# MiloszKrajewski/K4os.Compression.LZ4

Measured on AMD Instinct MI355X. Metric: GiB/s encode+decode on batched 64 KiB blocks; bit-exact vs C# ref, higher is better.
Workload: dtype u8

## Files before the change

k4os/compression/lz4_amd/csrc/k4lz4_capi.hip:

```cpp
#include <hip/hip_runtime.h>
#include <stdint.h>
#include <stdio.h>
#include <stdlib.h>
#include <string.h>
#include <algorithm>
#include <atomic>
#include <memory>
#include <new>
#include <condition_variable>
#include <functional>
#include <map>
#include <mutex>
#include <string>
#include <thread>
#include <chrono>
#include <vector>

#include "../../../../include/k4lz4.h"
#include "k4lz4_decode.hpp"
#include "k4lz4_encode_fast.hpp"
#include "k4lz4_parse.hpp"
#include "k4lz4_pickle.hpp"
#include "k4lz4_segments.hpp"
#include "k4lz4_encode_hc.hpp"
// ... 62 lines not shown
    hipEvent_t ev_up[MAX_PARTS] = {}, ev_len[MAX_PARTS] = {};
    uint8_t *h_len = nullptr; size_t h_len_cap = 0;
    struct Pool *pool = nullptr, *pool_dl = nullptr;
    bool pool_failed = false, pool_dl_failed = false;
    int stage_threads = 7;
    uint32_t *d_pace = nullptr;
    uint32_t *d_status = nullptr;
    int split_pct = -1;
    bool no_pair = false;
    int direct_span_pct = 200;
    bool no_direct = false;
    int lds_floor_per_cu = 8;
    int cost_pct = 48;
    int dec_parts = 4, dec_parts_direct = 8;
    int last_decode_kernel = 0;
    int hop2_max_per_cu = 12;
    bool hc_cand_lds = true;
    int hc_cand_dynlds = 0;
    int hc_segs = 0;
    bool hc_chain_parts = true;
    int hc_mem_pct = 33;
    int pace_min_per_cu = 6;
    bool use_pace = true;
    bool prof_gtab = false;
    uint8_t *d_parse = nullptr; size_t d_parse_cap = 0;
    bool use_parse = true;
    bool parse_queue = false;
    bool hc_records = true;
    bool parse_seg = true;
    bool parse_big = true;
    bool parse_persist = true;
    bool parse_inline_emit = true;
    bool parse_migrate = true;
    bool parse_pcost = false;
    int parse_waves = 16;
    bool trace = false;
    std::vector<uint8_t> h_chain;
    uint8_t *d_chain = nullptr; size_t d_chain_cap = 0;
    hipEvent_t ev_chain = nullptr;
    uint8_t *d_fr = nullptr; size_t d_fr_cap = 0;
    uint8_t *d_fb = nullptr; size_t d_fb_cap = 0;
    uint8_t *d_lg = nullptr; size_t d_lg_cap = 0;
    uint8_t *d_frd = nullptr; size_t d_frd_cap = 0;
    uint8_t *d_lgr = nullptr; size_t d_lgr_cap = 0;
    uint8_t *d_lga = nullptr; size_t d_lga_cap = 0;
    std::vector<uint8_t> h_fw;
    uint8_t *d_fw = nullptr; size_t d_fw_cap = 0;
    hipEvent_t ev_fw = nullptr;
    struct DictScratch {
        std::vector<uint8_t> host;
        uint8_t *dev = nullptr; size_t cap = 0;
        hipEvent_t ev = nullptr;
        std::vector<uint32_t> table, kept;
    } dict_fast, dict_hc;
    uint8_t *d_dpick = nullptr; size_t d_dpick_cap = 0;
};

struct k4lz4_dict_set {
    struct Family {
        bool on = false;
        uint64_t *toff = nullptr, *eoff = nullptr;
        uint32_t *tlen = nullptr, *elen = nullptr, *etab = nullptr;
        uint8_t *tables = nullptr;
        std::vector<uint32_t> table, kept;
        int64_t ntables = 0, loads = 0;
    };
    int device = -1;
// ... 413 lines not shown
                K4_HIP(ctx, hipStreamSynchronize(stream));
                K4_HIP(ctx, hipStreamSynchronize(ctx->aux2));
            }
            int rc = grow(ctx, &ctx->d_seg, &ctx->d_seg_cap, total, false);
            if (rc == K4LZ4_OK) rc = grow(ctx, &ctx->d_seg_first, &ctx->d_seg_first_cap, (size_t)cnt * 4, false);
            if (rc != K4LZ4_OK) return rc;
            sg.hdr = (k4::SegHdr *)ctx->d_seg; sg.items = (k4::SegItem *)(ctx->d_seg + o_items); sg.work = (uint32_t *)(ctx->d_seg + o_work);
            sg.blocks = (uint32_t *)(ctx->d_seg + o_blocks); sg.snaps = (uint32_t *)(ctx->d_seg + o_snaps); sg.tables = (uint32_t *)(ctx->d_seg + o_tables);
            sg.first = (int32_t *)ctx->d_seg_first;
            sg.seg_min = ctx->seg_min; sg.seg_target = ctx->seg_target; sg.seg_warm = ctx->seg_warm; sg.seg_div = ctx->seg_div; sg.seg_target_max = ctx->seg_target_max; sg.spin_max = ctx->seg_spin_max; sg.max_items = (uint32_t)max_items;
            hipLaunchKernelGGL(k4::k4_seg_plan_kernel, dim3(1), dim3(256), 0, stream, a, sg);
            a.seg_first = sg.first; a.seg_items = sg.items; a.seg_snaps = sg.snaps;
            seg = true;
        }
        auto segments_start = [&]() -> int {
            if (!seg) return K4LZ4_OK;
            K4_HIP(ctx, hipEventRecord(ctx->ev_fork, stream));
            K4_HIP(ctx, hipStreamWaitEvent(ctx->aux2, ctx->ev_fork, 0));
            hipLaunchKernelGGL(k4::k4_encode_seg_kernel, dim3((unsigned)((sg.max_items + k4::ENCODE_WAVES_PER_WG - 1) / k4::ENCODE_WAVES_PER_WG)), dim3(64 * k4::ENCODE_WAVES_PER_WG), 0, ctx->aux2, a, sg);
            K4_HIP(ctx, hipEventRecord(ctx->ev_join2, ctx->aux2));
            return K4LZ4_OK;
        };
        auto segments_join = [&]() -> int {
            if (!seg) return K4LZ4_OK;
            K4_HIP(ctx, hipStreamWaitEvent(stream, ctx->ev_join2, 0));
            hipLaunchKernelGGL(k4::k4_seg_join_kernel, dim3((unsigned)std::min<int64_t>(k4::SEG_MAX_BLOCKS, cnt)), dim3(64), 0, stream, a, sg);
            return K4LZ4_OK;
        };
        if (dd && dd->dict) {
            a.dict = dd->dict; a.dictOff = dd->off + first; a.dictLen = dd->len + first;
            a.dictMode = dd->mode ? dd->mode + first : nullptr;
        }
        if (reorder && parse_path && kind == KIND_ENCODE && ctx->parse_pcost) {
            a.cost = d_cost; a.hist = d_hist; a.order_out = d_order;
            K4_HIP(ctx, hipMemsetAsync(d_hist, 0, 2 * k4::PCOST_BUCKETS * 4, stream));
            hipLaunchKernelGGL(k4::k4_pcost_kernel, dim3((unsigned)((cnt + k4::PCOST_WAVES_PER_WG - 1) / k4::PCOST_WAVES_PER_WG)), dim3(64 * k4::PCOST_WAVES_PER_WG), 0, stream, a);
            hipLaunchKernelGGL(k4::k4_porder_kernel, dim3((unsigned)((cnt + 255) / 256)), dim3(256), 0, stream, a);
            a.order = d_order;
        }
        else if (reorder) {
            a.cost = d_cost; a.hist = d_hist; a.order_out = d_order;
            K4_HIP(ctx, hipMemsetAsync(d_hist, 0, (2 * k4::COST_BUCKETS + 16) * 4, stream));
            hipLaunchKernelGGL(k4::k4_cost_kernel, dim3((unsigned)cnt), dim3(64), 0, stream, a, encode_like ? 0 : 1,
                               kind == KIND_ENCODE && parse_path ? k4::COST_SAMPLE_PARSE : k4::COST_SAMPLE);
            const bool two_kernels = kind == KIND_ENCODE && !a.prof && cnt > 512 && !(flags & K4LZ4_FLAG_NO_SPLIT) &&
                                     cnt > 8 * (int64_t)ctx->cu_count && ctx->split_pct <= 0;
            k4::BatchArgs ao = a;
            ao.first = two_kernels ? (uint32_t)ctx->cost_pct : 0u;
            ao.total = (uint32_t)((int64_t)ctx->lds_floor_per_cu * (int64_t)ctx->cu_count);
            hipLaunchKernelGGL(k4::k4_order_kernel, dim3((unsigned)((cnt + 255) / 256)), dim3(256), 0, stream, ao, (uint32_t)lds_share(ctx, cnt));
            a.order = d_order;
            if (two_kernels) a.split = d_hist + 2 * k4::COST_BUCKETS;
        }
        const unsigned wg4 = (unsigned)((cnt + k4::DECODE_WAVES_PER_WG - 1) / k4::DECODE_WAVES_PER_WG);
        bool parse_here = kind == KIND_ENCODE && (parse_path || (parse_seg_path && (a.order || cnt == 1)));
        const bool big_ok = ctx->parse_big && ctx->parse_inline_emit;
        bool any_small = true, any_big = big_ok;
        if (parse_here && hostLen) {
            any_small = false; any_big = false;
            for (int64_t i = 0; i < cnt && !(any_small && (any_big || !big_ok)); i++) {
                const int32_t len = hostLen[first + i];
                if (len >= (int32_t)k4::PARSE_MIN_LEN && len < k4::LIMIT_64K) any_small = true;
                else if (len >= k4::LIMIT_64K && big_ok) any_big = true;
            }
            parse_here = any_small || any_big;
        }
        int64_t waves = 0, nwg = 0, nwg_seg = 0;
        const bool seg_two_step = seg && parse_here && parse_seg_path;
        bool queue = false, slot_recs = false;
        size_t o_meta = 0, o_gtab = 0;
// ... 1761 lines not shown
    if (e == hipSuccess) e = hipStreamCreateWithFlags(&ctx->dlq, hipStreamNonBlocking);
    if (const char *pct = getenv("K4LZ4_SPLIT_PCT")) { const int v = atoi(pct); ctx->split_pct = v < 1 ? 1 : (v > 100 ? 100 : v); }
    ctx->no_pair = getenv("K4LZ4_NO_PAIR") != nullptr;
    ctx->prof_gtab = getenv("K4LZ4_PROF_GTAB") != nullptr;
    ctx->use_pace = getenv("K4LZ4_NO_PACE") == nullptr;
    if (const char *e = getenv("K4LZ4_PACE_MIN")) ctx->pace_min_per_cu = std::max(0, atoi(e));
    if (const char *e = getenv("K4LZ4_DIRECT_SPAN_PCT")) ctx->direct_span_pct = std::max(100, atoi(e));
    if (const char *e = getenv("K4LZ4_NO_DIRECT")) ctx->no_direct = atoi(e) != 0;
    if (const char *e = getenv("K4LZ4_LDS_FLOOR")) ctx->lds_floor_per_cu = std::max(0, std::min(8, atoi(e)));
    if (const char *e = getenv("K4LZ4_COST_PCT")) ctx->cost_pct = std::max(1, std::min(99, atoi(e)));
    if (const char *e = getenv("K4LZ4_DEC_PARTS")) ctx->dec_parts = std::max(2, std::min(MAX_PARTS, atoi(e)));
    if (const char *e = getenv("K4LZ4_DEC_PARTS_DIRECT")) ctx->dec_parts_direct = std::max(2, std::min(MAX_PARTS, atoi(e)));
    if (const char *e = getenv("K4LZ4_HOP2_MAX")) ctx->hop2_max_per_cu = std::max(0, atoi(e));
    ctx->hc_chain_parts = getenv("K4LZ4_HC_CHAIN_OLD") == nullptr;
    ctx->hc_cand_lds = getenv("K4LZ4_HC_CAND_MEM") == nullptr;
    if (const char *e = getenv("K4LZ4_HC_CAND_DYNLDS")) ctx->hc_cand_dynlds = std::max(0, std::min(65536, atoi(e)));
    if (const char *e = getenv("K4LZ4_HC_SEGS")) { const int v = atoi(e); ctx->hc_segs = v >= 4 ? 4 : (v >= 2 ? 2 : (v == 1 ? 1 : 0)); }
    if (const char *e = getenv("K4LZ4_HC_MEM_PCT")) ctx->hc_mem_pct = std::max(0, std::min(100, atoi(e)));
    ctx->use_segments = getenv("K4LZ4_NO_SEGMENTS") == nullptr;
    if (const char *e = getenv("K4LZ4_SEG_MIN")) ctx->seg_min = (uint32_t)std::max(65536 + 4096, atoi(e));
    if (const char *e = getenv("K4LZ4_SEG_TARGET")) ctx->seg_target = ctx->seg_target_max = (uint32_t)std::max(8192, atoi(e));
    if (const char *e = getenv("K4LZ4_SEG_TARGET_MAX")) ctx->seg_target_max = (uint32_t)std::max(8192, atoi(e));
    if (const char *e = getenv("K4LZ4_SEG_WARM")) ctx->seg_warm = (uint32_t)std::max(0, atoi(e));
    if (const char *e = getenv("K4LZ4_SEG_SPIN_MAX")) ctx->seg_spin_max = (uint32_t)std::max(0, atoi(e));
    if (const char *e = getenv("K4LZ4_SEG_DIV")) ctx->seg_div = (uint32_t)std::max(0, atoi(e));
    if (const char *e = getenv("K4LZ4_PICKLE_SPLIT_MIN")) ctx->pickle_split_min = std::max(0, atoi(e));
    if (const char *e = getenv("K4LZ4_STAGE_THREADS")) ctx->stage_threads = std::max(0, std::min(63, atoi(e) - 1));
    ctx->use_parse = getenv("K4LZ4_NO_PARSE") == nullptr;
    ctx->parse_queue = getenv("K4LZ4_PARSE_QUEUE") != nullptr;
    ctx->parse_persist = getenv("K4LZ4_NO_PERSIST") == nullptr;
    ctx->parse_big = getenv("K4LZ4_NO_PARSE_BIG") == nullptr;
    ctx->parse_seg = getenv("K4LZ4_NO_PARSE_SEG") == nullptr;
    ctx->hc_records = getenv("K4LZ4_NO_HC_RECORDS") == nullptr;
    ctx->parse_pcost = getenv("K4LZ4_PCOST") != nullptr;
    ctx->parse_migrate = getenv("K4LZ4_NO_MIGRATE") == nullptr;
    ctx->parse_inline_emit = getenv("K4LZ4_NO_INLINE_EMIT") == nullptr;
    if (const char *e = getenv("K4LZ4_PARSE_WAVES")) ctx->parse_waves = std::max(1, std::min(k4::PARSE_MAX_WAVES, atoi(e)));
    ctx->trace = getenv("K4LZ4_TRACE") != nullptr;
    if (e != hipSuccess) { delete ctx; return hip_fail(nullptr, e, "hipStreamCreate"); }
    *out = ctx;
    return K4LZ4_OK;
}

void k4lz4_ctx_destroy(k4lz4_ctx *ctx)
{
    if (!ctx) return;
    (void)hipSetDevice(ctx->device);
    if (ctx->stream) { (void)hipStreamSynchronize(ctx->stream); (void)hipStreamDestroy(ctx->stream); }
    if (ctx->aux) { (void)hipStreamSynchronize(ctx->aux); (void)hipStreamDestroy(ctx->aux); }
    if (ctx->aux2) { (void)hipStreamSynchronize(ctx->aux2); (void)hipStreamDestroy(ctx->aux2); }
    if (ctx->ev_join2) (void)hipEventDestroy(ctx->ev_join2);
    if (ctx->d_seg) (void)hipFree(ctx->d_seg);
    if (ctx->d_seg_first) (void)hipFree(ctx->d_seg_first);
    if (ctx->ev_fork) (void)hipEventDestroy(ctx->ev_fork);
    if (ctx->ev_join) (void)hipEventDestroy(ctx->ev_join);
    if (ctx->ev_busy) (void)hipEventDestroy(ctx->ev_busy);
    for (int b = 0; b < 2; b++) {
        if (ctx->ev_in[b]) (void)hipEventDestroy(ctx->ev_in[b]);
        if (ctx->ev_out[b]) (void)hipEventDestroy(ctx->ev_out[b]);
        if (ctx->h_in[b]) (void)hipHostFree(ctx->h_in[b]);
        if (ctx->h_out[b]) (void)hipHostFree(ctx->h_out[b]);
    }
    if (ctx->d_pack) (void)hipFree(ctx->d_pack);
    if (ctx->h_len) (void)hipHostFree(ctx->h_len);
    for (int b = 0; b < MAX_PARTS; b++) {
        if (ctx->ev_up[b]) (void)hipEventDestroy(ctx->ev_up[b]);
        if (ctx->ev_len[b]) (void)hipEventDestroy(ctx->ev_len[b]);
// ... 2436 lines not shown
```

k4os/compression/lz4_amd/csrc/k4lz4_encode_fast.hpp:

```cpp
#pragma once
#include "k4lz4_common.hpp"

namespace k4 {

#ifndef K4_SEG_WAVES_MIN
#define K4_SEG_WAVES_MIN 5
#endif
#ifndef K4_GTAB_DUTY
#define K4_GTAB_DUTY 3
#endif
#ifndef K4_PACE
#define K4_PACE 1
#endif

template <int TYPE> struct FastTable;

template <> struct FastTable<1> {
    uint16_t *t;
    __device__ __forceinline__ static uint32_t hash(const uint8_t *p) { return (ld32u(p) * 2654435761u) >> (32 - 13); }
    __device__ __forceinline__ static uint32_t hash_of(uint32_t seq, uint32_t) { return (seq * 2654435761u) >> (32 - 13); }
    __device__ __forceinline__ uint32_t get(uint32_t h) const { return t[h]; }
    __device__ __forceinline__ void put(uint32_t h, uint32_t pos) const { t[h] = (uint16_t)pos; }
    __device__ __forceinline__ uint32_t get_nt(uint32_t h) const
    {
// ... 750 lines not shown
        op += last_run;
    }
    if (seq_count) *seq_count = sequences;
    if (sr) { sr->stop = U; sr->state = 2u; }
    if (PROF && pc && lane == 0) {
        pc[0] = prof_now<PROF>() - t_begin; pc[1] = c_probe; pc[2] = c_ext; pc[3] = c_emit;
        pc[4] = n_seq; pc[5] = n_round; pc[6] = n_dup; pc[7] = n_rt3;
        pc[11] = c_s1; pc[12] = c_s2; pc[13] = c_s3; pc[14] = c_s4; pc[15] = n_cont;
    }
    prof_place<PROF>(pc, 9, lane);
    return (int)op;
}

template <bool PAIRS = true, bool MORE = false, bool N2 = true, bool GTAB = false>
__device__ __forceinline__ int compress_fast_block(const uint8_t *src, int src_len, uint8_t *dst, int dst_cap,
                                                   int accel, uint32_t *ldsw, int lane, uint32_t *gtab = nullptr, bool x32 = false,
                                                   uint32_t *pace = nullptr, SegRun *sr = nullptr)
{
    const uint32_t a = accel < 1 ? 1u : (accel > 65536 ? 65536u : (uint32_t)accel);
    if (src_len < LIMIT_64K) return encode_fast_block<true, false, false, PAIRS, MORE, N2, GTAB>(src, src_len, dst, dst_cap, a, ldsw, lane, nullptr, false, nullptr, gtab, pace);
    if (x32) return encode_fast_block<false, false, true, PAIRS, MORE, N2, GTAB>(src, src_len, dst, dst_cap, a, ldsw, lane, nullptr, false, nullptr, gtab, pace, sr);
    return encode_fast_block<false, false, false, PAIRS, MORE, N2, GTAB>(src, src_len, dst, dst_cap, a, ldsw, lane, nullptr, false, nullptr, gtab, pace, sr);
}

__device__ __forceinline__ int codec_encode_result(int src_len, int ret, int flags)
{
    if (flags & FLAG_RAW_RETURN) return ret;
    if (src_len <= 0) return 0;
    return ret <= 0 ? -1 : ret;
}

constexpr int COST_SAMPLE = 512, COST_SAMPLE_PARSE = 256;
constexpr int COST_BUCKETS = 64;

__device__ __forceinline__ uint32_t cost_bucket(unsigned long long cost)
{
    if (cost < 4ull) return (uint32_t)cost;
    const uint32_t l = 63u - (uint32_t)__clzll(cost);
    const uint32_t bkt = 2u * l + (uint32_t)((cost >> (l - 1u)) & 1ull);
    return bkt < (uint32_t)COST_BUCKETS ? bkt : (uint32_t)COST_BUCKETS - 1u;
}

__global__ __launch_bounds__(64) void k4_cost_kernel(BatchArgs a, int by_length, int sample_bytes = COST_SAMPLE)
{
    __shared__ __attribute__((aligned(16))) uint32_t tab[ENCODE_LDS_DWORDS];
    const int lane = lane_id();
    const long long b = (long long)blockIdx.x;
    const int src_len = a.srcLen[b];
    unsigned long long cost = 0;
    if (src_len > 0) {
        if (by_length || src_len <= 64) {
            cost = (unsigned long long)src_len;
        } else {
            const int sample = src_len < sample_bytes ? src_len : sample_bytes;
            uint32_t nseq = 0;
            (void)encode_fast_block<true>(a.src + a.srcOff[b], sample, nullptr, 0x7fffffff, 1u, tab, lane, nullptr, true, &nseq);
            cost = ((unsigned long long)(nseq * 8u + (uint32_t)sample / 16u) * (unsigned long long)src_len) / (unsigned long long)sample;
        }
    }
    if (lane == 0) {
        const uint32_t bkt = cost_bucket(cost);
        a.cost[b] = bkt;
        atomicAdd(&a.hist[bkt], 1u);
    }
}

__device__ __forceinline__ unsigned long long bucket_cost(uint32_t bkt)
{
    if (bkt < 4u) return bkt ? (unsigned long long)bkt * 4ull : 1ull;
    const uint32_t l = bkt >> 1;
    return ((bkt & 1u) ? 7ull : 5ull) << (l - 1u);
}

__global__ __launch_bounds__(256) void k4_order_kernel(BatchArgs a, uint32_t lds_max = 0xffffffffu)
{
    if (blockIdx.x == 0 && threadIdx.x == 0 && a.first != 0u) {
        unsigned long long all = 0;
        for (uint32_t k = 0; k < (uint32_t)COST_BUCKETS; k++) all += (unsigned long long)a.hist[k] * bucket_cost(k);
        const unsigned long long want = all / 100ull * (unsigned long long)a.first;
        unsigned long long have = 0, cnt = 0;
        for (int k = COST_BUCKETS - 1; k >= 0 && have < want; k--) {
            const unsigned long long c = a.hist[k], w = bucket_cost((uint32_t)k);
            if (have + c * w <= want) { have += c * w; cnt += c; }
            else { const unsigned long long part = (want - have + w - 1ull) / w; cnt += part; have = want; }
        }
        const unsigned long long floor_n = (unsigned long long)a.total < (unsigned long long)a.n ? (unsigned long long)a.total : (unsigned long long)a.n;
        if (cnt < floor_n) cnt = floor_n;
        if (cnt > (unsigned long long)a.n) cnt = (unsigned long long)a.n;
        if (cnt > (unsigned long long)lds_max) cnt = (unsigned long long)lds_max;
        a.hist[2 * COST_BUCKETS] = (uint32_t)cnt;
    }
    const long long b = (long long)blockIdx.x * 256 + threadIdx.x;
    if (b >= a.n) return;
    const uint32_t bkt = a.cost[b];
    uint32_t before = 0;
    for (uint32_t k = bkt + 1u; k < (uint32_t)COST_BUCKETS; k++) before += a.hist[k];
    const uint32_t pos = before + atomicAdd(&a.hist[COST_BUCKETS + bkt], 1u);
    a.order_out[pos] = (uint32_t)b;
}

constexpr int ENCODE_WAVES_PER_WG = 2;
struct SegFirst { SegRun run; uint32_t cap; bool cut; };
__device__ __forceinline__ SegFirst seg_first_of(const BatchArgs &a, long long b)
{
    SegFirst f;
    f.cut = false; f.cap = 0u;
    f.run.begin = 0u; f.run.emit_from = 0u; f.run.stop_at = SEG_NONE; f.run.snap_pub = nullptr; f.run.snap_chk = nullptr; f.run.resume = nullptr;
    f.run.cut = 0u; f.run.stop = 0u; f.run.state = 3u; f.run.spin_max = 0u; f.run.fix = nullptr;
    if (!a.seg_first) return f;
    const int32_t it = (int32_t)uni((uint32_t)a.seg_first[b]);
    if (it < 0) return f;
    const uint32_t *w = (const uint32_t *)a.seg_items + SEG_ITEM_WORDS * (uint32_t)it;
    f.cut = true;
    f.run.spin_max = uni(((const uint32_t *)a.seg_items)[-(int)SEG_HDR_DWORDS + 3]);
    f.run.stop_at = uni(w[4]);
    f.cap = f.run.stop_at;
    f.run.snap_chk = a.seg_snaps + (size_t)(it + 1) * SEG_SNAP_DWORDS;
    f.run.fix = a.seg_snaps + (size_t)uni(((const uint32_t *)a.seg_items)[-(int)SEG_HDR_DWORDS + 7]) * SEG_SNAP_DWORDS + 4096ull * (unsigned long long)it;
    return f;
}
__device__ __forceinline__ void seg_first_done(const BatchArgs &a, long long b, const SegFirst &f, int ret, int lane)
{
    if (!f.cut || lane != 0) return;
    uint32_t *w = (uint32_t *)a.seg_items + SEG_ITEM_WORDS * (uint32_t)a.seg_first[b];
    w[6] = f.run.cut; w[7] = f.run.stop; w[8] = ret > 0 ? f.run.state : 3u; w[9] = (uint32_t)ret;
}

template <bool MORE, bool SEG = false>
__device__ __forceinline__ void encode_fast_kernel_body(const BatchArgs &a, uint32_t (*tabs)[ENCODE_LDS_DWORDS])
{
    const int lane = lane_id();
// ... 101 lines not shown
```

k4os/compression/lz4_amd/csrc/k4lz4_parse.hpp:

```cpp
#pragma once
#include "k4lz4_encode_fast.hpp"
#include <type_traits>
#ifdef K4_PARSE_DEBUG
#include <stdio.h>
#include <stdlib.h>
#endif

namespace k4 {

#ifndef K4_PARSE_K
#define K4_PARSE_K 1
#endif

constexpr uint32_t PARSE_REC_STRIDE = 16448u;
static_assert(PARSE_REC_STRIDE >= ((uint32_t)LIMIT_64K - 1u - 6u) / 4u + 1u + 62u, "a block below LIMIT_64K has at most (LIMIT_64K - 1 - 6) / 4 sequences; a round adds at most 64 / 4 + 1");
constexpr uint32_t PARSE_MIN_LEN = 128u;
constexpr uint32_t PARSE_REST = 0xffffffffu;
constexpr uint32_t PARSE_BIG = 0xfffffffeu;
constexpr int PARSE_MAX_WAVES = 16;
constexpr int PARSE_LDS_TABLES = 9;
constexpr int PARSE_SEEN_DWORDS = 128;

constexpr int PARSE_LDS_DWORDS = 4096 * PARSE_LDS_TABLES + PARSE_SEEN_DWORDS * PARSE_MAX_WAVES + 4;

// ... 34 lines not shown
}

__device__ __forceinline__ uint32_t ext28(const uint32_t *x)
{
    uint32_t acc = min((uint32_t)(__ffs((int)x[6]) - 1), 32u);
#pragma unroll
    for (int i = 5; i >= 0; i--) {
        const uint32_t t = min((uint32_t)(__ffs((int)x[i]) - 1), 32u);
        acc = t + (t == 32u ? acc : 0u);
    }
    return acc >> 3;
}

__device__ __forceinline__ void rec_store(uint2 *r, uint32_t x, uint32_t y)
{
#if defined(K4_NT_RECS) && !defined(K4_HOST_EMU)
    __builtin_nontemporal_store((((unsigned long long)y) << 32) | x, (unsigned long long *)r);
#else
    *r = make_uint2(x, y);
#endif
}
__device__ __forceinline__ uint2 rec_load(const uint2 *r)
{
#if defined(K4_NT_RECS) && !defined(K4_HOST_EMU)
    const unsigned long long v = __builtin_nontemporal_load((const unsigned long long *)r);
    return make_uint2((uint32_t)v, (uint32_t)(v >> 32));
#else
    return *r;
#endif
}

constexpr uint32_t HOP_LONG = 0x100u, HOP_LAZY = 0x200u, HOP_END = 0x400u, HOP_INVALID = 0x800u, HOP_TABMISS = 0x1000u;

struct ParseStats { uint32_t rounds, slow, groups, lazies, longs; };
constexpr int PARSE_FLUSH = -2;

struct ParseCtl {
    uint32_t *free_slots;
    uint32_t rec_cap;
    int claimed;
    bool resume;
    uint32_t c, sbase, sj, nrec, long_seen, long_rounds;
    bool test, more;
    uint32_t cut_pos;
    bool dry, stopped;
};

template <int K, bool GT, bool DRY = false, int TT = 1, bool SEG = false>
__device__ __forceinline__ uint32_t parse_block(const uint8_t *src, const uint32_t U, uint2 *recs, void *tabv, uint32_t *seen, const int lane, unsigned long long *pc = nullptr,
                                                ParseStats *stats = nullptr, ParseCtl *ctl = nullptr, SegRun *sr = nullptr)
{
    static_assert(!SEG || (TT != 1 && K == 1 && !DRY), "segments: byU32 blocks, one sub-window per round");
    typedef FastTable<TT> Table;
    static_assert(TT == 1 || K == 1, "byU32 tables: one sub-window per round");
    constexpr bool U32 = TT != 1;
    Table tab;
    tab.t = (decltype(tab.t))tabv;
    constexpr uint32_t SEEN_SHIFT = TT == 1 ? 1u : 0u;
    ParseStats st = {0u, 0u, 0u, 0u, 0u};
#define K4_ST(field, v) do { if (DRY) st.field += (v); } while (0)
#ifdef K4_PARSE_PROF
    unsigned long long pt[8] = {0, 0, 0, 0, 0, 0, 0, 0}, pn[8] = {0, 0, 0, 0, 0, 0, 0, 0}, plast = 0;
    const unsigned long long pbegin = prof_now<true>();
#define K4_PT(i) do { const unsigned long long t_ = prof_now<true>(); pt[i] += t_ - plast; plast = t_; } while (0)
#define K4_PN(i, v) (pn[i] += (v))
#define K4_TIC() const unsigned long long tic_ = (unsigned long long)__builtin_readcyclecounter()
#define K4_TOC(i) (pt[i] += (unsigned long long)__builtin_readcyclecounter() - tic_)
#else
#define K4_TIC() ((void)0)
#define K4_TOC(i) ((void)0)
#define K4_PT(i) ((void)0)
#define K4_PN(i, v) ((void)0)
#endif
#if defined(K4_PARSE_PROF) && !defined(K4_PARSE_PROF_SPLIT)
#define K4_TICA() K4_TIC()
#define K4_TOCA(i) K4_TOC(i)
#else
#define K4_TICA() ((void)0)
#define K4_TOCA(i) ((void)0)
#endif
#if defined(K4_PARSE_PROF) && defined(K4_PARSE_PROF_SPLIT)
#define K4_TICB() const unsigned long long ticb_ = (unsigned long long)__builtin_readcyclecounter()
#define K4_TOCB(i) (pt[i] += (unsigned long long)__builtin_readcyclecounter() - ticb_)
#define K4_TICC() const unsigned long long ticc_ = (unsigned long long)__builtin_readcyclecounter()
#define K4_TOCC(i) (pt[i] += (unsigned long long)__builtin_readcyclecounter() - ticc_)
#else
#define K4_TICB() ((void)0)
#define K4_TOCB(i) ((void)0)
#define K4_TICC() ((void)0)
#define K4_TOCC(i) ((void)0)
#endif
    const uint32_t mfl1 = U - (uint32_t)MFLIMIT + 1u;
// ... 671 lines not shown
    for (;;) {
        if (SEG) {
            cut_hit = uni(cut_hit ? 1u : 0u) != 0u;
            if (cut_hit) {
                cut_hit = false;
                if (handle_cut()) { ctl->stopped = true; return nrec; }
            }
            cut_pos = uni(cut_pos); nrec = uni(nrec); dry = uni(dry ? 1u : 0u) != 0u;
            c = uni(c); sbase = uni(sbase);
        }
        if (U32 && rec_cap && nrec + 64u * (uint32_t)K + 2u > rec_cap) {
            ctl->c = c; ctl->sbase = sbase; ctl->sj = sj; ctl->nrec = nrec; ctl->test = test; ctl->more = more;
            ctl->long_seen = long_seen; ctl->long_rounds = long_rounds;
            if (SEG) { ctl->cut_pos = cut_pos; ctl->dry = dry; }
            ctl->claimed = PARSE_FLUSH;
            return nrec;
        }
        if (GT && ctl && ctl->free_slots && (++mig_tick & 15u) == 0u) {
            const uint32_t fs = uni(lds_peek(ctl->free_slots));
            if (fs) {
                const uint32_t sl = (uint32_t)__ffs((int)fs) - 1u;
                uint32_t old = 0u;
                if (lane == 0) old = atomicAnd(ctl->free_slots, ~(1u << sl));
                if (uni(old) & (1u << sl)) {
                    ctl->c = c; ctl->sbase = sbase; ctl->sj = sj; ctl->nrec = nrec; ctl->test = test; ctl->more = more;
                    ctl->long_seen = long_seen; ctl->long_rounds = long_rounds;
                    if (SEG) { ctl->cut_pos = cut_pos; ctl->dry = dry; }
                    ctl->claimed = (int)sl;
                    wave_sync();
                    return nrec;
                }
            }
        }
        const bool plain = sj == 0u && c + 64u * (uint32_t)K + 28u <= U;
        if (K == 1 && plain && c + 63u <= sbase + 65u) {
            if (more && c + 108u <= U) { if (!fast_round(std::true_type{})) break; }
            else if (!fast_round(std::false_type{})) break;
        }
        else if (plain) { if (!round(std::true_type{})) break; }
        else if (!round(std::false_type{})) break;
    }
#ifdef K4_PARSE_PROF
    if (pc && lane == 0) {
        pc[0] = prof_now<true>() - pbegin;
        for (int i = 0; i < 6; i++) pc[1 + i] = pt[i];
        pc[7] = (unsigned long long)nrec | (pn[4] << 32);
        pc[11] = pn[0] | (pn[6] << 32);
        pc[12] = pn[1] | (pn[2] << 32);
        pc[13] = (pt[6] & 0xffffffffull) | (pt[7] << 32);
        pc[10] = pn[7];
        pc[14] = pn[3] | (pn[5] << 32);
    }
#endif
    if (DRY && stats) *stats = st;
#undef K4_ST
    if (SEG) {
        if (uni(dry ? 1u : 0u) != 0u) {
            agent_publish(sr->snap_pub, SEG_NONE);
            sr->state = 3u;
            ctl->stopped = true;
            nrec = 0u;
        } else {
            sr->stop = U; sr->state = 2u;
        }
    }
    return nrec;
// ... 128 lines not shown
        const bool mine = a.accel == 1 && (U32 ? big : (src_len >= (int)PARSE_MIN_LEN && src_len < LIMIT_64K));
        if (!mine) {
            if (!U32 && lane == 0) {
                meta[0] = (big && p.big) ? PARSE_BIG : PARSE_REST; meta[1] = 0u;
                if (big && p.big && p.nbig) atomicAdd(p.nbig, 1u);
            }
        } else {
            uint32_t n = 0u;
            const int ret = parse_one<K, TT, false>(a, p, lds, seen, in_lds, wave, waves, lane, b, a.src + a.srcOff[b], src_len, a.dst + a.dstOff[b], a.dstCap[b], nullptr, &n);
            if (lane == 0) {
                meta[0] = n; meta[1] = 0u;
                if (p.inline_emit) a.outLen[b] = codec_encode_result(src_len, ret, a.flags);
            }
        }
        if (!p.queue) return;
    }
}


__global__ __launch_bounds__(64 * PARSE_MAX_WAVES) void k4_parse_kernel(BatchArgs a, ParseArgs p)
{
    __shared__ __attribute__((aligned(16))) uint32_t lds[PARSE_LDS_DWORDS];
    parse_kernel_body<K4_PARSE_K>(a, p, lds);
}

__global__ __launch_bounds__(64 * PARSE_MAX_WAVES) void k4_parse_big_kernel(BatchArgs a, ParseArgs p)
{
    __shared__ __attribute__((aligned(16))) uint32_t lds[PARSE_LDS_DWORDS];
    if (a.flags & FLAG_X32) parse_kernel_body<1, 2>(a, p, lds);
    else parse_kernel_body<1, 0>(a, p, lds);
}


constexpr uint32_t PCOST_SAMPLE = 3072u;
constexpr int PCOST_BUCKETS = 512;
constexpr int PCOST_WAVES_PER_WG = 8;

__device__ __forceinline__ uint32_t pcost_bucket(unsigned long long cost)
{
    if (cost < 256ull) return 0u;
    const uint32_t l = 63u - (uint32_t)__clzll((long long)cost);
    const uint32_t b = 16u * (l - 8u) + (uint32_t)((cost >> (l - 4u)) & 15ull) + 1u;
    return b < (uint32_t)PCOST_BUCKETS ? b : (uint32_t)PCOST_BUCKETS - 1u;
}

__global__ __launch_bounds__(64 * PCOST_WAVES_PER_WG) void k4_pcost_kernel(BatchArgs a)
{
    __shared__ __attribute__((aligned(16))) uint32_t lds[PCOST_WAVES_PER_WG][4096 + PARSE_SEEN_DWORDS];
    const int lane = lane_id();
    const uint32_t wave = uni(threadIdx.x >> 6);
    const long long b = (long long)blockIdx.x * PCOST_WAVES_PER_WG + (long long)wave;
    if (b >= a.n) return;
    const int src_len = a.srcLen[b];
    unsigned long long cost = 0ull;
    if (src_len >= (int)PARSE_MIN_LEN && src_len < LIMIT_64K) {
        const uint32_t sample = (uint32_t)src_len < PCOST_SAMPLE ? (uint32_t)src_len : PCOST_SAMPLE;
        ParseStats st;
        const uint32_t nseq = parse_block<1, false, true>(a.src + a.srcOff[b], sample, nullptr, (uint16_t *)lds[wave], lds[wave] + 4096, lane, nullptr, &st);
        const unsigned long long cyc = 6500ull * st.rounds + 3000ull * st.slow + 120ull * nseq + 150ull * st.groups + 480ull * st.lazies + 1500ull * st.longs;
        cost = cyc * (unsigned long long)(uint32_t)src_len / sample;
    } else if (src_len > 0) {
        cost = 120ull * (unsigned long long)(uint32_t)src_len;
    }
    if (lane == 0) {
        const uint32_t bkt = pcost_bucket(cost);
        a.cost[b] = bkt;
        atomicAdd(&a.hist[bkt], 1u);
    }
}

__global__ __launch_bounds__(256) void k4_porder_kernel(BatchArgs a)
{
    __shared__ uint32_t before[PCOST_BUCKETS];
    for (int k = (int)threadIdx.x; k < PCOST_BUCKETS; k += 256) before[k] = a.hist[k];
    __syncthreads();
    if (threadIdx.x == 0) {
        uint32_t acc = 0u;
        for (int k = PCOST_BUCKETS - 1; k >= 0; k--) { const uint32_t c = before[k]; before[k] = acc; acc += c; }
    }
    __syncthreads();
    const long long b = (long long)blockIdx.x * 256 + threadIdx.x;
    if (b >= a.n) return;
    const uint32_t bkt = a.cost[b];
    a.order_out[before[bkt] + atomicAdd(&a.hist[PCOST_BUCKETS + bkt], 1u)] = (uint32_t)b;
}


constexpr int EMIT_WAVES_PER_WG = 4;

template <bool HC, bool BIG>
__device__ __forceinline__ bool emit_records(const uint8_t *src, const uint32_t U, uint8_t *dst, const int dst_cap, const uint2 *recs, const uint32_t nseq, const int lane, EmitState &st)
{
    const bool limited = dst_cap < compress_bound((int)U);
    const uint64_t olimit = (uint64_t)(dst_cap < 0 ? 0 : dst_cap);
    uint32_t op = st.op, emitted_to = st.emitted_to;
    uint2 rn = make_uint2(0u, 0u);
    if ((uint32_t)lane < nseq) rn = rec_load(recs + lane);
    for (uint32_t base = 0u; base < nseq; base += 64u) {
        const uint32_t n = nseq - base < 64u ? nseq - base : 64u;
        const bool mine = (uint32_t)lane < n;
        const uint2 r = rn;
        if (base + 64u + (uint32_t)lane < nseq) rn = rec_load(recs + base + 64u + (uint32_t)lane);
        const uint32_t pos = r.x, cpos = r.x - (r.y & 0xffffu);
        uint32_t code = r.y >> 16;
        if (BIG) {
            unsigned long long lng = ballot(mine && code == 0xffffu);
            while (lng) {
                const int g = ctz64(lng);
                lng &= lng - 1ull;
                const uint32_t gp = readlane_u32(pos, g), gc = readlane_u32(cpos, g);
                const uint32_t full = wave_count(src + gp + (uint32_t)MINMATCH, src + gc + (uint32_t)MINMATCH, (U - (uint32_t)LASTLITERALS) - (gp + (uint32_t)MINMATCH), lane);
                if (lane == g) code = full;
            }
        }
        const uint32_t end = mine ? pos + (uint32_t)MINMATCH + code : 0u;
        const uint32_t prev = (uint32_t)__shfl_up((int)end, 1);
        const uint32_t ls = lane == 0 ? emitted_to : prev;
        const uint32_t lit0 = mine ? pos - ls : 0u;
// ... 140 lines not shown
```

Measured before the change: 61.55.

## Enable fitted parse-cost ordering by default with persistent cost kernel

Turns on the parse-based cost estimate for ordering encode work by default. It replaces the old pcost kernel with a persistent grid-stride kernel that uses LDS plus global-memory hash tables and a round cap. It also takes cost weights fitted offline from measured per-block timings and switches the order kernel to a wave-scan suffix count over fine buckets. The aim is to schedule expensive blocks first and reduce tail imbalance. The cost is an extra sampling pass before every encode, and the fitted weights may not carry over to other data.

```diff
diff --git a/experiments/parse_cost_order/fit.py b/experiments/parse_cost_order/fit.py
--- /dev/null
+++ b/experiments/parse_cost_order/fit.py
@@ -0,0 +1,68 @@
+import ctypes as C, os, sys, subprocess, numpy as np
+ROOT = os.path.dirname(os.path.dirname(os.path.dirname(os.path.abspath(__file__))))
+sys.path.insert(0, ROOT)
+WORK = sys.argv[1]
+from k4os.compression.lz4_amd import corpus
+so = os.path.join(WORK, "libstudy.so")
+lib = C.CDLL(so)
+n, bs = 4096, 65536
+cache = os.path.join(WORK, "blocks.npy")
+if os.path.exists(cache): blocks = np.load(cache)
+else:
+    blocks = corpus.silesia_like_blocks(n, bs, seed=2); np.save(cache, blocks)
+uidx = np.array([ci + 12 * t for ci in range(12) for t in range(32)])
+ub = np.ascontiguousarray(blocks[uidx])
+off = (np.arange(384, dtype=np.uint64) * bs); lens = np.full(384, bs, np.int32)
+def stats(o, l):
+    out = np.zeros((384, 8), np.uint32)
+    lib.study_stats(ub.ctypes.data_as(C.POINTER(C.c_uint8)), C.c_void_p(off.ctypes.data), C.c_void_p(lens.ctypes.data), C.c_longlong(384), C.c_uint32(o), C.c_uint32(l), C.c_void_p(out.ctypes.data), C.c_int(8), C.c_uint32(0))
+    return out[:, :6].astype(np.float64), out[:, 6].astype(np.float64)
+b = np.arange(n); u = (b % 12) * 32 + (b // 12) % 32
+ls = np.zeros(384); ln = np.zeros(384); ms = np.zeros(384); mn = np.zeros(384)
+for f in ("parent_blocks", "oracleP_blocks", "oracleQ_blocks"):
+    res = np.load(os.path.join(WORK, "%s.npy" % f))
+    for r in res:
+        d = (r[:, 1] - r[:, 0]) / 1e5; k = r[:, 2].astype(int)
+        np.add.at(ls, u[k == 4], d[k == 4]); np.add.at(ln, u[k == 4], 1)
+        np.add.at(ms, u[k != 4], d[k != 4]); np.add.at(mn, u[k != 4], 1)
+lds = np.where(ln > 0, ls / np.maximum(ln, 1), np.nan); mem = np.where(mn > 0, ms / np.maximum(mn, 1), np.nan)
+both = (ln >= 2) & (mn >= 2)
+ratio = np.median(mem[both] / lds[both]); print("ratio", ratio, "both", both.sum(), "lds known", (ln > 0).sum())
+truth = np.where(np.isnan(lds), mem / ratio, lds)
+np.save(os.path.join(WORK, "truth.npy"), truth)
+names = corpus.SILESIA_NAMES
+def evaluate(tag, est):
+    e = est[u] + 1e-9 * np.random.default_rng(0).random(n)
+    t = truth[u]
+    cut = np.sort(e)[::-1][2303]
+    inl = e >= cut
+    tail_mem = (t[~inl] * ratio).max(); tail_lds = t[inl].max()
+    tcut = np.sort(t)[::-1][2303]
+    mis = ((t >= tcut) & ~inl).sum()
+    from scipy.stats import spearmanr
+    rho = spearmanr(est, truth).correlation
+    print("%-28s rho %.3f misplaced %4d  tail mem %.3f lds %.3f  mem>2.7: %4d  mem>2.85: %4d" % (tag, rho, mis, tail_mem, tail_lds, (t[~inl] * ratio > 2.7).sum(), (t[~inl] * ratio > 2.85).sum()))
+evaluate("truth", truth)
+full, _ = stats(0, 65536)
+np.save(os.path.join(WORK, "full.npy"), full)
+for ci, nm in enumerate(names):
+    s = full[ci * 32:(ci + 1) * 32]
+    print("%-8s truth %.3f | rounds %6.0f slow %6.0f nseq %6.0f groups %6.0f lazies %6.0f longs %6.0f" % ((nm, truth[ci * 32:(ci + 1) * 32].mean()) + tuple(s.mean(0))))
+A = np.c_[full, np.ones(384)]
+w, *_ = np.linalg.lstsq(A, truth, rcond=None)
+print("fit full (ms per unit):", w, "resid rms", np.sqrt(((A @ w - truth) ** 2).mean()))
+from scipy.optimize import nnls
+w2, _ = nnls(A, truth); print("nnls:", w2, "rms", np.sqrt(((A @ w2 - truth) ** 2).mean()))
+evaluate("full stats, lstsq", A @ w)
+evaluate("full stats, nnls", A @ w2)
+evaluate("full stats, old pcost w", full @ np.array([6500, 3000, 120, 150, 480, 1500.]))
+evaluate("full rounds only", full[:, 0])
+for (o, l) in ((0, 256), (0, 512), (0, 1024), (0, 2048), (0, 3072), (32768, 512), (32768, 1024), (16384, 1024), (4096, 1024), (1024, 1024)):
+    s, sl = stats(o, l)
+    sc = s * (bs / sl)[:, None]
+    evaluate("sample %d+%d nnls-w" % (o, l), np.c_[sc, np.ones(384)] @ w2)
+    evaluate("sample %d+%d lstsq-w" % (o, l), np.c_[sc, np.ones(384)] @ w)
+    evaluate("sample %d+%d oldw" % (o, l), sc @ np.array([6500, 3000, 120, 150, 480, 1500.]))
+    As = np.c_[sc, np.ones(384)]; ws, _ = nnls(As, truth)
+    evaluate("sample %d+%d refit" % (o, l), As @ ws); print("    refit w", np.round(ws, 6))
+    np.save(os.path.join(WORK, "s_%d_%d.npy" % (o, l)), sc)
diff --git a/experiments/parse_cost_order/fit_stats.cpp b/experiments/parse_cost_order/fit_stats.cpp
--- /dev/null
+++ b/experiments/parse_cost_order/fit_stats.cpp
@@ -0,0 +1,30 @@
+#include "hip/hip_runtime.h"
+#include "k4lz4_decode.hpp"
+#include "k4lz4_encode_fast.hpp"
+#include "k4lz4_parse.hpp"
+#include <vector>
+
+namespace k4 {
+__global__ void stats_kernel(BatchArgs a, uint32_t off, uint32_t len, uint32_t *out, uint32_t cap = 0)
+{
+    __shared__ __attribute__((aligned(16))) uint32_t lds[PCOST_WAVES_PER_WG][4096 + PARSE_SEEN_DWORDS];
+    const int lane = lane_id();
+    const uint32_t wave = uni(threadIdx.x >> 6);
+    const long long b = (long long)blockIdx.x * PCOST_WAVES_PER_WG + (long long)wave;
+    if (b >= a.n) return;
+    const uint32_t src_len = (uint32_t)a.srcLen[b];
+    uint32_t o = off, s = len;
+    if (o + s > src_len) { o = 0; s = s < src_len ? s : src_len; }
+    ParseStats st; st.max_rounds = cap;
+    const uint32_t nseq = parse_block<1, false, true>(a.src + a.srcOff[b] + o, s, nullptr, (uint16_t *)lds[wave], lds[wave] + 4096, lane, nullptr, &st);
+    if (lane == 0) { uint32_t *w = out + 8 * b; w[0] = st.rounds; w[1] = st.slow; w[2] = nseq; w[3] = st.groups; w[4] = st.lazies; w[5] = st.longs; w[6] = st.covered; }
+}
+}
+
+extern "C" int study_stats(const uint8_t *src, const uint64_t *srcOff, const int32_t *srcLen, long long n, uint32_t off, uint32_t len, uint32_t *out, int threads, uint32_t cap)
+{
+    k4::BatchArgs a{};
+    a.src = src; a.srcOff = srcOff; a.srcLen = srcLen; a.n = n; a.accel = 1;
+    k4emu::launch_fn(dim3((unsigned)((n + k4::PCOST_WAVES_PER_WG - 1) / k4::PCOST_WAVES_PER_WG)), dim3(64 * k4::PCOST_WAVES_PER_WG), [=] { k4::stats_kernel(a, off, len, out, cap); }, threads);
+    return 0;
+}
diff --git a/experiments/parse_cost_order/rank_blocks.py b/experiments/parse_cost_order/rank_blocks.py
--- /dev/null
+++ b/experiments/parse_cost_order/rank_blocks.py
@@ -0,0 +1,26 @@
+#!/usr/bin/env python
+import sys
+import numpy as np
+res = np.load(sys.argv[1])
+reps, n, _ = res.shape
+b = np.arange(n)
+u = (b % 12) * 32 + (b // 12) % 32
+dur = (res[:, :, 1] - res[:, :, 0]) / 1e5
+k = res[:, :, 2].astype(int)
+lds_s = np.zeros(384); lds_n = np.zeros(384); mem_s = np.zeros(384); mem_n = np.zeros(384)
+for r in range(reps):
+    np.add.at(lds_s, u[k[r] == 4], dur[r][k[r] == 4]); np.add.at(lds_n, u[k[r] == 4], 1)
+    np.add.at(mem_s, u[k[r] != 4], dur[r][k[r] != 4]); np.add.at(mem_n, u[k[r] != 4], 1)
+lds = np.where(lds_n > 0, lds_s / np.maximum(lds_n, 1), np.nan)
+mem = np.where(mem_n > 0, mem_s / np.maximum(mem_n, 1), np.nan)
+both = (lds_n >= 2) & (mem_n >= 2)
+ratio = float(np.median(mem[both] / lds[both])) if both.any() else 1.17
+P = np.where(np.isnan(lds), mem / ratio, lds)
+Q = np.where(np.isnan(mem), lds * ratio, mem)
+print("unique blocks with LDS stamps %d, with others %d, with both %d; ratio other / LDS %.3f" % ((lds_n > 0).sum(), (mem_n > 0).sum(), both.sum(), ratio))
+for tag, est, path in (("P", P, sys.argv[2]), ("Q", Q, sys.argv[3])):
+    bkt = np.clip(np.round(est / (est.max() * 1.0001) * 63.0), 0, 63).astype(np.uint8)
+    bkt[u].tofile(path)
+    cut = np.sort(est[u])[::-1][2304 - 1]
+    print("%s: estimate ms min %.3f max %.3f; the 2304th most expensive block has %.3f; LDS share per class:" % (tag, est.min(), est.max(), cut),
+          " ".join("%d:%.2f" % (c, float((est[u][c::12] >= cut).mean())) for c in range(12)))
diff --git a/experiments/parse_cost_order/rank_from_stamp.py b/experiments/parse_cost_order/rank_from_stamp.py
--- /dev/null
+++ b/experiments/parse_cost_order/rank_from_stamp.py
@@ -0,0 +1,29 @@
+#!/usr/bin/env python
+import re, sys
+NAMES = ("dickens", "mozilla", "mr", "nci", "ooffice", "osdb", "reymont", "samba", "sao", "webster", "xml", "x-ray")
+lds, mem = {}, {}
+kern, on = None, False
+for line in open(sys.argv[1]):
+    if line.startswith("ENCODE"): on = True; continue
+    if line.startswith("DECODE"): on = False
+    if not on: continue
+    m = re.match(r"\s*kernel (\d+) blocks", line)
+    if m: kern = int(m.group(1)); continue
+    m = re.match(r"\s*(\S+)\s+n\s+(\d+)\s+start.*duration mean ([\d.]+)", line)
+    if m and kern is not None:
+        name, cnt, d = m.group(1), int(m.group(2)), float(m.group(3))
+        if kern == 4: lds[name] = (cnt, d)
+        elif kern in (5, 6):
+            c0, d0 = mem.get(name, (0, 0.0))
+            mem[name] = (c0 + cnt, (c0 * d0 + cnt * d) / (c0 + cnt))
+both = sorted(mem[k][1] - lds[k][1] for k in NAMES if k in lds and k in mem and lds[k][0] >= 8 and mem[k][0] >= 8)
+pen = both[len(both) // 2] if both else 0.4
+estA, estB = {}, {}
+for k in NAMES:
+    estA[k] = lds[k][1] if k in lds and lds[k][0] >= 8 else max(0.0, mem[k][1] - pen)
+    estB[k] = mem[k][1] if k in mem and mem[k][0] >= 8 else lds[k][1] + pen
+for tag, est in (("A", estA), ("B", estB)):
+    ranked = sorted(NAMES, key=lambda k: est[k])
+    rank = {k: i for i, k in enumerate(ranked)}
+    print("%s=%s" % (tag, ",".join(str(rank[k]) for k in NAMES)))
+    print("# %s penalty %.3f most expensive first: %s" % (tag, pen, "  ".join("%s %.3f" % (k, est[k]) for k in reversed(ranked))), file=sys.stderr)
diff --git a/experiments/parse_cost_order/stamp_dump.py b/experiments/parse_cost_order/stamp_dump.py
--- /dev/null
+++ b/experiments/parse_cost_order/stamp_dump.py
@@ -0,0 +1,43 @@
+#!/usr/bin/env python
+import os, sys
+import numpy as np
+import torch
+sys.path.insert(0, os.getcwd())
+from k4os.compression.lz4_amd import LZ4Codec, corpus
+from k4os.compression.lz4_amd.device import DeviceBatch, DeviceCodec
+
+out, reps = sys.argv[1], int(sys.argv[2]) if len(sys.argv) > 2 else 4
+n, bs = 4096, 65536
+blocks = corpus.silesia_like_blocks(n, bs, seed=2)
+dc = DeviceCodec(0)
+lens = np.full(n, bs, np.int32)
+off = np.arange(n, dtype=np.uint64) * bs
+src = DeviceBatch.from_host(blocks.reshape(-1), off, lens, dc.device)
+comp = DeviceBatch.empty_slots(np.full(n, LZ4Codec.MaximumOutputSize(bs)), dc.device)
+dc.encode(src, comp)
+torch.cuda.synchronize()
+res = []
+for rep in range(reps + 1):
+    _, c = dc.profile(4, src, comp)
+    torch.cuda.synchronize()
+    c = c.cpu().numpy().astype(np.float64)
+    if rep: res.append(np.stack([c[:, 8], c[:, 9], c[:, 11], c[:, 12]], axis=1))
+res = np.stack(res)
+np.save(out, res)
+for r in res:
+    st, en, k = r[:, 0], r[:, 1], r[:, 2].astype(int)
+    t0 = st.min()
+    print("span ms %.3f | LDS n %d last end %.3f | memory n %d last end %.3f | moved n %d last end %.3f" % (
+        (en.max() - t0) / 1e5, (k == 4).sum(), (en[k == 4].max() - t0) / 1e5, (k == 5).sum(), (en[k == 5].max() - t0) / 1e5 if (k == 5).any() else 0,
+        (k == 6).sum(), (en[k == 6].max() - t0) / 1e5 if (k == 6).any() else 0))
+names = corpus.SILESIA_NAMES
+r = res[-1]
+k = r[:, 2].astype(int)
+for ci, name in enumerate(names):
+    idx = np.arange(ci, n, 12)
+    d = (r[idx, 1] - r[idx, 0]) / 1e5
+    kk = k[idx]
+    print("  %-8s LDS %3d mem %3d moved %3d | dur LDS mean %.3f max %.3f | not-LDS mean %.3f max %.3f | end max %.3f" % (
+        name, (kk == 4).sum(), (kk == 5).sum(), (kk == 6).sum(),
+        d[kk == 4].mean() if (kk == 4).any() else 0, d[kk == 4].max() if (kk == 4).any() else 0,
+        d[kk != 4].mean() if (kk != 4).any() else 0, d[kk != 4].max() if (kk != 4).any() else 0, (r[idx, 1].max() - r[:, 0].min()) / 1e5))
diff --git a/k4os/compression/lz4_amd/csrc/k4lz4_capi.hip b/k4os/compression/lz4_amd/csrc/k4lz4_capi.hip
--- a/k4os/compression/lz4_amd/csrc/k4lz4_capi.hip
+++ b/k4os/compression/lz4_amd/csrc/k4lz4_capi.hip
@@ -118,7 +118,8 @@
     bool parse_persist = true;
     bool parse_inline_emit = true;
     bool parse_migrate = true;
-    bool parse_pcost = false;
+    bool parse_pcost = true;
+    k4::ParseCost pcost_fit = k4::PCOST_FIT;
     int parse_waves = 16;
     bool trace = false;
     std::vector<uint8_t> h_chain;
@@ -598,10 +599,17 @@
             a.dictMode = dd->mode ? dd->mode + first : nullptr;
         }
         if (reorder && parse_path && kind == KIND_ENCODE && ctx->parse_pcost) {
+            const int64_t wgs = std::min<int64_t>((cnt + k4::PARSE_MAX_WAVES - 1) / k4::PARSE_MAX_WAVES, ctx->cu_count);
+            const size_t need = (size_t)wgs * (k4::PARSE_MAX_WAVES - k4::PARSE_LDS_TABLES) * 16384;
+            if (need > ctx->d_parse_cap) K4_HIP(ctx, hipStreamSynchronize(stream));
+            const int rcp = grow(ctx, &ctx->d_parse, &ctx->d_parse_cap, need, false);
+            if (rcp != K4LZ4_OK) return rcp;
             a.cost = d_cost; a.hist = d_hist; a.order_out = d_order;
             K4_HIP(ctx, hipMemsetAsync(d_hist, 0, 2 * k4::PCOST_BUCKETS * 4, stream));
-            hipLaunchKernelGGL(k4::k4_pcost_kernel, dim3((unsigned)((cnt + k4::PCOST_WAVES_PER_WG - 1) / k4::PCOST_WAVES_PER_WG)), dim3(64 * k4::PCOST_WAVES_PER_WG), 0, stream, a);
-            hipLaunchKernelGGL(k4::k4_porder_kernel, dim3((unsigned)((cnt + 255) / 256)), dim3(256), 0, stream, a);
+            k4::ParseCost pc = ctx->pcost_fit;
+            pc.tables = (uint32_t *)ctx->d_parse;
+            hipLaunchKernelGGL(static_cast<void (*)(k4::BatchArgs, k4::ParseCost)>(k4::k4_cost_kernel), dim3((unsigned)wgs), dim3(64 * k4::PARSE_MAX_WAVES), 0, stream, a, pc);
+            hipLaunchKernelGGL(k4::k4_order_kernel, dim3((unsigned)((cnt + 255) / 256)), dim3(256), 0, stream, a, 0xffffffffu, 1);
             a.order = d_order;
         }
         else if (reorder) {
@@ -2429,7 +2437,12 @@
     ctx->parse_big = getenv("K4LZ4_NO_PARSE_BIG") == nullptr;
     ctx->parse_seg = getenv("K4LZ4_NO_PARSE_SEG") == nullptr;
     ctx->hc_records = getenv("K4LZ4_NO_HC_RECORDS") == nullptr;
-    ctx->parse_pcost = getenv("K4LZ4_PCOST") != nullptr;
+    ctx->parse_pcost = getenv("K4LZ4_NO_PCOST") == nullptr || getenv("K4LZ4_PCOST") != nullptr;
+    if (const char *e = getenv("K4LZ4_PCOST_FIT")) {
+        unsigned v[9];
+        if (sscanf(e, "%u,%u,%u,%u,%u,%u,%u,%u,%u", &v[0], &v[1], &v[2], &v[3], &v[4], &v[5], &v[6], &v[7], &v[8]) == 9 && v[0] >= k4::PARSE_MIN_LEN && v[0] < 65536u)
+            ctx->pcost_fit = k4::ParseCost{v[0], v[1], v[2], v[3], v[4], v[5], v[6], v[7], v[8], nullptr};
+    }
     ctx->parse_migrate = getenv("K4LZ4_NO_MIGRATE") == nullptr;
     ctx->parse_inline_emit = getenv("K4LZ4_NO_INLINE_EMIT") == nullptr;
     if (const char *e = getenv("K4LZ4_PARSE_WAVES")) ctx->parse_waves = std::max(1, std::min(k4::PARSE_MAX_WAVES, atoi(e)));
diff --git a/k4os/compression/lz4_amd/csrc/k4lz4_encode_fast.hpp b/k4os/compression/lz4_amd/csrc/k4lz4_encode_fast.hpp
--- a/k4os/compression/lz4_amd/csrc/k4lz4_encode_fast.hpp
+++ b/k4os/compression/lz4_amd/csrc/k4lz4_encode_fast.hpp
@@ -806,6 +806,7 @@
 
 constexpr int COST_SAMPLE = 512, COST_SAMPLE_PARSE = 256;
 constexpr int COST_BUCKETS = 64;
+constexpr int COST_BUCKETS_FINE = 512;
 
 __device__ __forceinline__ uint32_t cost_bucket(unsigned long long cost)
 {
@@ -846,8 +847,40 @@
     return ((bkt & 1u) ? 7ull : 5ull) << (l - 1u);
 }
 
-__global__ __launch_bounds__(256) void k4_order_kernel(BatchArgs a, uint32_t lds_max = 0xffffffffu)
-{
+template <int NB>
+__device__ __forceinline__ void suffix_counts(const uint32_t *hist, uint32_t *before, uint32_t *above)
+{
+    static_assert(NB % 64 == 0 && NB <= 4096, "whole waves of counts; their totals fit one wave");
+    const uint32_t lane = (uint32_t)lane_id(), wave = uni(threadIdx.x >> 6), waves = blockDim.x >> 6;
+    for (uint32_t c = wave; c < (uint32_t)NB / 64u; c += waves) {
+        const uint32_t k = (uint32_t)NB - 1u - (64u * c + lane);
+        const uint32_t v = hist[k], incl = wave_inclusive_scan(v);
+        before[k] = incl - v;
+        if (lane == 63u) above[c] = incl;
+    }
+    __syncthreads();
+    if (wave == 0u) {
+        const uint32_t v = lane < (uint32_t)NB / 64u ? above[lane] : 0u, incl = wave_inclusive_scan(v);
+        if (lane < (uint32_t)NB / 64u) above[lane] = incl - v;
+    }
+    __syncthreads();
+}
+
+template <int NB>
+__device__ __forceinline__ void order_by_bucket(const BatchArgs &a)
+{
+    __shared__ uint32_t before[NB], above[NB / 64];
+    suffix_counts<NB>(a.hist, before, above);
+    const long long b = (long long)blockIdx.x * 256 + threadIdx.x;
+    if (b >= a.n) return;
+    const uint32_t bkt = a.cost[b];
+    const uint32_t pos = before[bkt] + above[((uint32_t)NB - 1u - bkt) >> 6] + atomicAdd(&a.hist[NB + bkt], 1u);
+    a.order_out[pos] = (uint32_t)b;
+}
+
+__global__ __launch_bounds__(256) void k4_order_kernel(BatchArgs a, uint32_t lds_max = 0xffffffffu, int fine = 0)
+{
+    if (fine) { order_by_bucket<COST_BUCKETS_FINE>(a); return; }
     if (blockIdx.x == 0 && threadIdx.x == 0 && a.first != 0u) {
         unsigned long long all = 0;
         for (uint32_t k = 0; k < (uint32_t)COST_BUCKETS; k++) all += (unsigned long long)a.hist[k] * bucket_cost(k);
@@ -864,13 +897,7 @@
         if (cnt > (unsigned long long)lds_max) cnt = (unsigned long long)lds_max;
         a.hist[2 * COST_BUCKETS] = (uint32_t)cnt;
     }
-    const long long b = (long long)blockIdx.x * 256 + threadIdx.x;
-    if (b >= a.n) return;
-    const uint32_t bkt = a.cost[b];
-    uint32_t before = 0;
-    for (uint32_t k = bkt + 1u; k < (uint32_t)COST_BUCKETS; k++) before += a.hist[k];
-    const uint32_t pos = before + atomicAdd(&a.hist[COST_BUCKETS + bkt], 1u);
-    a.order_out[pos] = (uint32_t)b;
+    order_by_bucket<COST_BUCKETS>(a);
 }
 
 constexpr int ENCODE_WAVES_PER_WG = 2;
diff --git a/k4os/compression/lz4_amd/csrc/k4lz4_parse.hpp b/k4os/compression/lz4_amd/csrc/k4lz4_parse.hpp
--- a/k4os/compression/lz4_amd/csrc/k4lz4_parse.hpp
+++ b/k4os/compression/lz4_amd/csrc/k4lz4_parse.hpp
@@ -90,7 +90,7 @@
 
 constexpr uint32_t HOP_LONG = 0x100u, HOP_LAZY = 0x200u, HOP_END = 0x400u, HOP_INVALID = 0x800u, HOP_TABMISS = 0x1000u;
 
-struct ParseStats { uint32_t rounds, slow, groups, lazies, longs; };
+struct ParseStats { uint32_t rounds, slow, groups, lazies, longs; uint32_t covered, max_rounds; };
 constexpr int PARSE_FLUSH = -2;
 
 struct ParseCtl {
@@ -115,7 +115,7 @@
     Table tab;
     tab.t = (decltype(tab.t))tabv;
     constexpr uint32_t SEEN_SHIFT = TT == 1 ? 1u : 0u;
-    ParseStats st = {0u, 0u, 0u, 0u, 0u};
+    ParseStats st = {0u, 0u, 0u, 0u, 0u, U, DRY && stats ? uni(stats->max_rounds) : 0u};
 #define K4_ST(field, v) do { if (DRY) st.field += (v); } while (0)
 #ifdef K4_PARSE_PROF
     unsigned long long pt[8] = {0, 0, 0, 0, 0, 0, 0, 0}, pn[8] = {0, 0, 0, 0, 0, 0, 0, 0}, plast = 0;
@@ -853,6 +853,7 @@
                 }
             }
         }
+        if (DRY && st.max_rounds && uni(st.rounds) >= st.max_rounds) { st.covered = uni(c); break; }
         const bool plain = sj == 0u && c + 64u * (uint32_t)K + 28u <= U;
         if (K == 1 && plain && c + 63u <= sbase + 65u) {
             if (more && c + 108u <= U) { if (!fast_round(std::true_type{})) break; }
@@ -1047,58 +1048,69 @@
 }
 
 
-constexpr uint32_t PCOST_SAMPLE = 3072u;
-constexpr int PCOST_BUCKETS = 512;
-constexpr int PCOST_WAVES_PER_WG = 8;
+struct ParseCost {
+    uint32_t sample, max_rounds;
+    uint32_t round, slow, seq, group, lazy, lng;
+    uint32_t base;
+    uint32_t *tables;
+};
+constexpr ParseCost PCOST_FIT = {2048u, 10u, 999u, 0u, 104u, 0u, 18u, 181u, 835300u, nullptr};
+constexpr int PCOST_BUCKETS = COST_BUCKETS_FINE;
+constexpr int PCOST_WAVES_PER_WG = PARSE_MAX_WAVES;
 
 __device__ __forceinline__ uint32_t pcost_bucket(unsigned long long cost)
 {
-    if (cost < 256ull) return 0u;
+    if (cost < 16384ull) return 0u;
     const uint32_t l = 63u - (uint32_t)__clzll((long long)cost);
-    const uint32_t b = 16u * (l - 8u) + (uint32_t)((cost >> (l - 4u)) & 15ull) + 1u;
+    const uint32_t b = 32u * (l - 14u) + (uint32_t)((cost >> (l - 5u)) & 31ull) + 1u;
     return b < (uint32_t)PCOST_BUCKETS ? b : (uint32_t)PCOST_BUCKETS - 1u;
 }
 
-__global__ __launch_bounds__(64 * PCOST_WAVES_PER_WG) void k4_pcost_kernel(BatchArgs a)
-{
-    __shared__ __attribute__((aligned(16))) uint32_t lds[PCOST_WAVES_PER_WG][4096 + PARSE_SEEN_DWORDS];
+__device__ __forceinline__ void parse_cost_body(const BatchArgs &a, const ParseCost &pc, uint32_t *lds, uint32_t *far)
+{
     const int lane = lane_id();
     const uint32_t wave = uni(threadIdx.x >> 6);
-    const long long b = (long long)blockIdx.x * PCOST_WAVES_PER_WG + (long long)wave;
-    if (b >= a.n) return;
-    const int src_len = a.srcLen[b];
-    unsigned long long cost = 0ull;
-    if (src_len >= (int)PARSE_MIN_LEN && src_len < LIMIT_64K) {
-        const uint32_t sample = (uint32_t)src_len < PCOST_SAMPLE ? (uint32_t)src_len : PCOST_SAMPLE;
-        ParseStats st;
-        const uint32_t nseq = parse_block<1, false, true>(a.src + a.srcOff[b], sample, nullptr, (uint16_t *)lds[wave], lds[wave] + 4096, lane, nullptr, &st);
-        const unsigned long long cyc = 6500ull * st.rounds + 3000ull * st.slow + 120ull * nseq + 150ull * st.groups + 480ull * st.lazies + 1500ull * st.longs;
-        cost = cyc * (unsigned long long)(uint32_t)src_len / sample;
-    } else if (src_len > 0) {
-        cost = 120ull * (unsigned long long)(uint32_t)src_len;
-    }
-    if (lane == 0) {
-        const uint32_t bkt = pcost_bucket(cost);
-        a.cost[b] = bkt;
-        atomicAdd(&a.hist[bkt], 1u);
-    }
-}
-
-__global__ __launch_bounds__(256) void k4_porder_kernel(BatchArgs a)
-{
-    __shared__ uint32_t before[PCOST_BUCKETS];
-    for (int k = (int)threadIdx.x; k < PCOST_BUCKETS; k += 256) before[k] = a.hist[k];
-    __syncthreads();
-    if (threadIdx.x == 0) {
-        uint32_t acc = 0u;
-        for (int k = PCOST_BUCKETS - 1; k >= 0; k--) { const uint32_t c = before[k]; before[k] = acc; acc += c; }
-    }
-    __syncthreads();
-    const long long b = (long long)blockIdx.x * 256 + threadIdx.x;
-    if (b >= a.n) return;
-    const uint32_t bkt = a.cost[b];
-    a.order_out[before[bkt] + atomicAdd(&a.hist[PCOST_BUCKETS + bkt], 1u)] = (uint32_t)b;
-}
+    uint32_t *seen = lds + 4096u * (uint32_t)PARSE_LDS_TABLES + (uint32_t)PARSE_SEEN_DWORDS * wave;
+    for (long long b = (long long)blockIdx.x * PARSE_MAX_WAVES + (long long)wave; b < a.n; b += (long long)gridDim.x * PARSE_MAX_WAVES) {
+        const int src_len = a.srcLen[b];
+        unsigned long long cost = 0ull;
+        if (src_len >= (int)PARSE_MIN_LEN && src_len < LIMIT_64K) {
+            const uint32_t sample = (uint32_t)src_len < pc.sample ? (uint32_t)src_len : pc.sample;
+            const uint8_t *src = a.src + a.srcOff[b];
+            ParseStats st;
+            st.max_rounds = pc.max_rounds;
+            uint32_t nseq;
+            if (wave < (uint32_t)PARSE_LDS_TABLES) nseq = parse_block<1, false, true>(src, sample, nullptr, lds + 4096u * wave, seen, lane, nullptr, &st);
+            else nseq = parse_block<1, true, true>(src, sample, nullptr, far + 4096u * (wave - (uint32_t)PARSE_LDS_TABLES), seen, lane, nullptr, &st);
+            const unsigned long long ns = (unsigned long long)pc.round * st.rounds + (unsigned long long)pc.slow * st.slow + (unsigned long long)pc.seq * nseq +
+                                          (unsigned long long)pc.group * st.groups + (unsigned long long)pc.lazy * st.lazies + (unsigned long long)pc.lng * st.longs;
+            cost = ns * (unsigned long long)(uint32_t)src_len / (st.covered ? st.covered : 1u) + (((unsigned long long)pc.base * (unsigned long long)(uint32_t)src_len) >> 16);
+        } else if (src_len > 0) {
+            cost = 40ull * (unsigned long long)(uint32_t)src_len;
+        }
+        if (lane == 0) {
+            const uint32_t bkt = pcost_bucket(cost);
+            a.cost[b] = bkt;
+            atomicAdd(&a.hist[bkt], 1u);
+        }
+    }
+}
+
+__global__ __launch_bounds__(64 * PARSE_MAX_WAVES) void k4_cost_kernel(BatchArgs a, ParseCost pc)
+{
+    __shared__ __attribute__((aligned(16))) uint32_t lds[4096 * PARSE_LDS_TABLES + PARSE_SEEN_DWORDS * PARSE_MAX_WAVES];
+    parse_cost_body(a, pc, lds, pc.tables + 4096ull * (unsigned long long)(PARSE_MAX_WAVES - PARSE_LDS_TABLES) * (unsigned long long)blockIdx.x);
+}
+
+#ifdef K4_HOST_EMU
+inline void k4_pcost_kernel(BatchArgs a)
+{
+    __shared__ __attribute__((aligned(16))) uint32_t lds[4096 * PARSE_LDS_TABLES + PARSE_SEEN_DWORDS * PARSE_MAX_WAVES];
+    __shared__ __attribute__((aligned(16))) uint32_t far[4096 * (PARSE_MAX_WAVES - PARSE_LDS_TABLES)];
+    parse_cost_body(a, PCOST_FIT, lds, far);
+}
+inline void k4_porder_kernel(BatchArgs a) { k4_order_kernel(a, 0xffffffffu, 1); }
+#endif
 
 
 constexpr int EMIT_WAVES_PER_WG = 4;
```

After: 62.37, median of 6. +1.3%, better.
